# JuliaQuantumControl/Krotov.jl

Hardware: NVIDIA B200
Metric: state_timesteps_per_s (higher is better)
Workload: dtype f64

## Files before the change

krotov.jl_b200/csrc/krotov_cuda.cu:

```cuda
#include <cuda_runtime.h>

#include <algorithm>
#include <chrono>
#include <cmath>
#include <complex>
#include <cstdio>
#include <cstdlib>
#include <cstring>
#include <map>
#include <set>
#include <string>
#include <vector>

#include <thread>

#include "../../include/krotov_cuda.h"
#include "dense_kernel.cuh"
#include "warp_kernel.cuh"
#include "warp2_kernel.cuh"
#include "tiny_kernel.cuh"
#include "kernel_table.h"

using cplx = std::complex<double>;

// ... 961 lines not shown
            dst.assign((size_t)N * h->lpt, cplx(0, 0));
            const cplx *s = reinterpret_cast<const cplx *>(src);
            for (int k = 0; k < N; ++k)
                for (int i = 0; i < d; ++i) dst[(size_t)k * h->lpt + i] = s[(size_t)k * d + i];
        };
        std::vector<cplx> tmp;
        pad_states(pb->psi0, tmp);
        if ((rc = upload(h, h->d_psi0, tmp))) return bail(rc);
        if (h->has_target) {
            pad_states(pb->target, tmp);
            if ((rc = upload(h, h->d_target, tmp))) return bail(rc);
        }
        const size_t slab = (size_t)N * (N_T + 1) * h->lpt * 16;
        h->x_slab = slab / 16;
        if ((rc = dev_alloc(h, h->d_X, slab * (h->rf_wanted ? 2 : 1)))) return bail(rc);
        if (h->store_fw && (rc = dev_alloc(h, h->d_Phi, slab))) return bail(rc);
        if ((rc = dev_alloc(h, h->d_chiT, (size_t)N * h->lpt * 16))) return bail(rc);
        if ((rc = dev_alloc(h, h->d_psif, (size_t)N * h->lpt * 16))) return bail(rc);
        cudaMemcpy(h->d_psif.p, h->d_psi0.p, (size_t)N * h->lpt * 16, cudaMemcpyDeviceToDevice);
        if (h->has_target) {
            std::vector<cplx> tau0(N);
            const cplx *s0 = reinterpret_cast<const cplx *>(pb->psi0), *tg = reinterpret_cast<const cplx *>(pb->target);
            for (int k = 0; k < N; ++k) {
                cplx a(0, 0);
                for (int i = 0; i < d; ++i) a += std::conj(tg[(size_t)k * d + i]) * s0[(size_t)k * d + i];
                tau0[k] = a;
            }
            cudaMemcpy(h->d_tau.p, tau0.data(), (size_t)N * 16, cudaMemcpyHostToDevice);
        }
        h->swept = true;
        if ((rc = dev_alloc(h, h->d_R, ((size_t)N_T * h->nCTA * L + (size_t)N_T * L) * 8))) return bail(rc);
        if ((rc = dev_alloc(h, h->d_acc, (size_t)N_T * L * kr::kFixLimbs * 8))) return bail(rc);
        if (getenv("KROTOV_PROF")) {
            if ((rc = dev_alloc(h, h->d_prof, (size_t)h->nCTA * 8 * 8))) return bail(rc);
            cudaMemset(h->d_prof.p, 0, h->d_prof.bytes);
        }
    } else {
        kr::SparseDesc sd;
        if (path == KROTOV_PATH_SPARSE) {
            sd.W = hs.W; sd.nnz_union = hs.nnz_union; sd.hermitian = hs.hermitian;
            sd.cols = &hs.cols; sd.vals_f = &hs.vals_f; sd.vals_b = &hs.vals_b;
        }
        h->dense = kr::dense_create(h->d, h->N, h->L, h->N_T, h->n_gen, h->Hdense, h->gen_of_traj, pb->psi0,
                                    pb->target, h->store_fw, h->stream, h->err,
                                    path == KROTOV_PATH_SPARSE ? &sd : nullptr);
        if (!h->dense) return bail(KROTOV_ERR_UNSUPPORTED);
        std::vector<cplx>().swap(h->Hdense);
        if (!kr::dense_seed(h->dense, (double2 *)h->d_tau.p, h->err)) return bail(KROTOV_ERR_CUDA);
        h->swept = true;
    }
    if (cudaDeviceSynchronize() != cudaSuccess) return bail(fail(h, KROTOV_ERR_CUDA, "device sync after create failed"));
    *out = h;
    return KROTOV_OK;
}

int krotov_get_info(krotov_handle h, krotov_info *out) {
    if (!h || !out) return KROTOV_ERR_ARG;
    memset(out, 0, sizeof(*out));
    out->struct_size = sizeof(krotov_info);
    out->path = h->path;
    out->ell_width = h->Wt;
    out->nnz_union = h->nnz_union;
    out->grid_blocks = h->nCTA;
    out->block_threads = h->wpc * h->lpt + 32;
    if (h->tiny && h->world == 1 && !h->amp_set) {
        out->grid_blocks = 1;
        out->block_threads = 32;
// ... 505 lines not shown

int krotov_envelope_extremes_device(krotov_handle h, int n_corner, const double *amps, double *e_min, double *e_max) {
    if (!h) return KROTOV_ERR_ARG;
    if (n_corner < 1 || !amps || !e_min || !e_max) return fail(h, KROTOV_ERR_ARG, "bad argument to krotov_envelope_extremes_device");
    if (h->path != KROTOV_PATH_WARP || h->lpt != 32 || !h->d_rawf.p)
        return fail(h, KROTOV_ERR_UNSUPPORTED, "krotov_envelope_extremes_device: persistent kernel path with d <= 32 only");
    cudaSetDevice(h->device);
    int rc;
    const size_t n_out = (size_t)h->n_gen * n_corner;
    if ((rc = dev_alloc(h, h->d_envamps, (size_t)n_corner * h->L * 8 + 16))) return rc;
    if ((rc = dev_alloc(h, h->d_envout, n_out * 16))) return rc;
    KR_CUDA(h, cudaMemcpyAsync(h->d_envamps.p, amps, (size_t)n_corner * h->L * 8, cudaMemcpyHostToDevice, h->stream));
    jacobi_extremes_kernel<<<(unsigned)n_out, 32, 0, h->stream>>>((const double2 *)h->d_rawf.p, (const int *)h->d_cols.p,
                                                                  (const double *)h->d_envamps.p, (double2 *)h->d_envout.p,
                                                                  h->L, h->Wt, h->d, n_corner);
    std::vector<double> out(2 * n_out);
    KR_CUDA(h, cudaMemcpyAsync(out.data(), h->d_envout.p, n_out * 16, cudaMemcpyDeviceToHost, h->stream));
    KR_CUDA(h, cudaStreamSynchronize(h->stream));
    h->launches_total += 1;
    for (int g = 0; g < h->n_gen; ++g) {
        double lo = out[2 * ((size_t)g * n_corner)], hi = out[2 * ((size_t)g * n_corner) + 1];
        for (int c = 1; c < n_corner; ++c) {
            lo = std::min(lo, out[2 * ((size_t)g * n_corner + c)]);
            hi = std::max(hi, out[2 * ((size_t)g * n_corner + c) + 1]);
        }
        e_min[g] = lo;
        e_max[g] = hi;
    }
    return KROTOV_OK;
}

int krotov_get_profile(krotov_handle h, int cta, int64_t *out) {
    if (!h || !out) return KROTOV_ERR_ARG;
    for (int i = 0; i < 8; ++i) out[i] = 0;
    if (!h->d_prof.p) return fail(h, KROTOV_ERR_STATE, "profiling counters are off (set KROTOV_PROF=1 before krotov_create)");
    cudaSetDevice(h->device);
    std::vector<long long> tmp((size_t)h->nCTA * 8);
    KR_CUDA(h, cudaMemcpy(tmp.data(), h->d_prof.p, tmp.size() * 8, cudaMemcpyDeviceToHost));
    if (cta >= h->nCTA) return fail(h, KROTOV_ERR_ARG, "cta out of range");
    for (int c = 0; c < h->nCTA; ++c)
        if (cta < 0 || c == cta)
            for (int i = 0; i < 8; ++i) out[i] = std::max<int64_t>(out[i], tmp[(size_t)c * 8 + i]);
    return KROTOV_OK;
}

struct CommDesc {
    cudaIpcMemHandle_t mh[2];
    cudaIpcMemHandle_t xh;
};
struct CommDescTail {
    int nCTA;
    int n_traj, n_traj_global;
    int rf_ok;
};
static_assert(sizeof(CommDesc) + sizeof(CommDescTail) <= KROTOV_COMM_DESC_BYTES, "descriptor too large");

int krotov_comm_export(krotov_handle h, void *desc) {
    if (!h || !desc) return KROTOV_ERR_ARG;
    cudaSetDevice(h->device);
    CommDesc cd;
    memset(&cd, 0, sizeof(cd));
    for (int par = 0; par < 2; ++par) KR_CUDA(h, cudaIpcGetMemHandle(&cd.mh[par], h->d_mbox[par].p));
    if (h->path == KROTOV_PATH_WARP) KR_CUDA(h, cudaIpcGetMemHandle(&cd.xh, h->d_X.p));
    memset(desc, 0, KROTOV_COMM_DESC_BYTES);
    memcpy(desc, &cd, sizeof(cd));
    CommDescTail tail{h->path == KROTOV_PATH_WARP ? h->nCTA : 0, h->N, h->N_global, rf_eligible(h) ? 1 : 0};
    memcpy((char *)desc + sizeof(cd), &tail, sizeof(tail));
    return KROTOV_OK;
}

int krotov_comm_connect(krotov_handle h, int rank, int world, const void *descs) {
    if (!h || !descs) return KROTOV_ERR_ARG;
    if (world < 1 || world > kr::kMaxRanks || rank < 0 || rank >= world) return fail(h, KROTOV_ERR_ARG, "bad rank/world");
    cudaSetDevice(h->device);
    h->rank = rank;
// ... 54 lines not shown
```

krotov.jl_b200/csrc/warp2_kernel.cuh:

```cuda
#pragma once
#include "warp_kernel.cuh"

namespace kr {

template <int W>
__device__ __forceinline__ void row_dot2(const double2 (&g)[W + 1], const int (&col)[W], const double2 *__restrict__ va,
                                         const double2 *__restrict__ vb, const double2 owna, const double2 ownb,
                                         double &ara, double &aia, double &arb, double &aib) {
    double ra1 = 0.0, ia1 = 0.0, rb1 = 0.0, ib1 = 0.0;
    ara = fma(g[W].x, owna.x, ara);
    ra1 = fma(-g[W].y, owna.y, ra1);
    aia = fma(g[W].x, owna.y, aia);
    ia1 = fma(g[W].y, owna.x, ia1);
    arb = fma(g[W].x, ownb.x, arb);
    rb1 = fma(-g[W].y, ownb.y, rb1);
    aib = fma(g[W].x, ownb.y, aib);
    ib1 = fma(g[W].y, ownb.x, ib1);
#pragma unroll
    for (int s = 0; s < W; ++s) {
        const double2 xa = va[col[s]];
        const double2 xb = vb[col[s]];
        ara = fma(g[s].x, xa.x, ara);
        ra1 = fma(-g[s].y, xa.y, ra1);
        aia = fma(g[s].x, xa.y, aia);
// ... 39 lines not shown
        oai = fma(cj, aia, oai);
        obr = fma(cj, arb, obr);
        obi = fma(cj, aib, obi);
        a2 = a1; b2 = b1;
        a1 = make_double2(ara, aia);
        b1 = make_double2(arb, aib);
        nxtA[lane] = a1;
        nxtB[lane] = b1;
        __syncwarp();
        double2 *t = curA; curA = nxtA; nxtA = t;
        t = curB; curB = nxtB; nxtB = t;
    }
    psia = make_double2(phase.x * oar - phase.y * oai, phase.x * oai + phase.y * oar);
    psib = make_double2(phase.x * obr - phase.y * obi, phase.x * obi + phase.y * obr);
}

template <int W, int LT>
__global__ void __launch_bounds__(256, 1) krotov_warp2_kernel(const __grid_constant__ WarpParams p) {
    constexpr int NT = 1 + LT;
    extern __shared__ __align__(16) unsigned char smem_raw[];
    const int lane = threadIdx.x & 31;
    const int warp = threadIdx.x >> 5;
    constexpr int L = LT;
    const int wpc = p.wpc;
    double2 *vbuf = reinterpret_cast<double2 *>(smem_raw);
    double2 *psis = vbuf + (size_t)wpc * 128;
    double *red = reinterpret_cast<double *>(psis + (size_t)wpc * 64);
    double *eps_s = red + (size_t)L * wpc * 32;
    double *gbuf = eps_s + kMaxCtrl;
    const int nthr_all = (wpc + 1) * 32;
    const int N_T = p.N_T;
    if (warp == wpc) {
        __shared__ __align__(16) WarpParams p_sh;
        comm_warp_run(p, (int)blockIdx.x, L, lane, wpc, nthr_all, red, eps_s, gbuf, &p_sh);
        return;
    }
    const int ka = (blockIdx.x * wpc + warp) * 2, kb = ka + 1;
    const bool live = kb < p.N;
    double2 *bufs = vbuf + (size_t)warp * 128;
    double2 *myps = psis + (size_t)warp * 64;
    int col[W];
#pragma unroll
    for (int s = 0; s < W; ++s) col[s] = p.cols[s * 32 + lane];
    const size_t rowstride = (size_t)(W + 1) * 32;
    double2 P[NT][W + 1];
    double2 g[W + 1];
    const int gi = live ? p.gen_of_traj[ka] : 0;
    const long long t_begin = clock64();

    if (p.mode == 1 && live) {
        const double2 *Pg = p.Pb + (size_t)gi * NT * rowstride;
#pragma unroll
        for (int q = 0; q < NT; ++q) load_row<W>(Pg + q * rowstride, P[q], lane);
        double2 ca, cb;
        if (p.chiT != nullptr) {
            ca = p.chiT[(size_t)ka * 32 + lane];
            cb = p.chiT[(size_t)kb * 32 + lane];
        } else {
            const double2 fa = p.chi_coef[ka], fb = p.chi_coef[kb];
            const double2 ta = p.target[(size_t)ka * 32 + lane], tb = p.target[(size_t)kb * 32 + lane];
            ca = make_double2(fa.x * ta.x - fa.y * ta.y, fa.x * ta.y + fa.y * ta.x);
            cb = make_double2(fb.x * tb.x - fb.y * tb.y, fb.x * tb.y + fb.y * tb.x);
        }
        double2 *Xa = p.X + (size_t)ka * (N_T + 1) * 32, *Xb = p.X + (size_t)kb * (N_T + 1) * 32;
        Xa[(size_t)N_T * 32 + lane] = ca;
        Xb[(size_t)N_T * 32 + lane] = cb;
        myps[lane] = ca;
// ... 92 lines not shown
            for (int l = 0; l < LT; ++l) eps[l] = p.amp_old[(size_t)l * N_T + n];
        }
        const StepMeta fmeta_next =
            load_meta(p.dtc_f, p.m_f, p.phase_f, p.coef_f, p.ndtc_f, p.mmax_f, gi, n + 1 < N_T ? n + 1 : n);
        if (live) {
#pragma unroll
            for (int s = 0; s <= W; ++s) g[s] = P[0][s];
#pragma unroll
            for (int l = 0; l < LT; ++l) {
#pragma unroll
                for (int s = 0; s <= W; ++s) {
                    g[s].x = fma(eps[l], P[l + 1][s].x, g[s].x);
                    g[s].y = fma(eps[l], P[l + 1][s].y, g[s].y);
                }
            }
            cheby_step2<W>(pa, pb, g, col, myps, bufs, fmeta.a, fmeta.m, fmeta.phase, lane);
            myps[lane] = pa;
            myps[32 + lane] = pb;
            __syncwarp();
            if (p.store_fw) {
                const int slot = (p.mode == 1) ? n : n + 1;
                p.Phi[((size_t)ka * (N_T + 1) + slot) * 32 + lane] = pa;
                p.Phi[((size_t)kb * (N_T + 1) + slot) * 32 + lane] = pb;
            }
        }
        fmeta = fmeta_next;
        if (p.prof != nullptr) {
            asm volatile("" ::"d"(pa.x) : "memory");
            t_step += clock64() - ts0;
        }
    }
    if (p.prof != nullptr && warp == 0 && lane == 0) {
        const long long t_end = clock64();
        p.prof[blockIdx.x * 8 + 0] = t_bw_end - t_begin;
        p.prof[blockIdx.x * 8 + 1] = t_end - t_bw_end;
        p.prof[blockIdx.x * 8 + 2] = t_wait_b;
        p.prof[blockIdx.x * 8 + 6] = t_overlap;
        p.prof[blockIdx.x * 8 + 7] = t_step;
    }
    if (live) {
        p.psi_final[(size_t)ka * 32 + lane] = pa;
        p.psi_final[(size_t)kb * 32 + lane] = pb;
        double tar = 0.0, tai = 0.0, tbr = 0.0, tbi = 0.0;
        if (p.target != nullptr) {
            const double2 ta = p.target[(size_t)ka * 32 + lane], tb = p.target[(size_t)kb * 32 + lane];
            tar = ta.x * pa.x + ta.y * pa.y;
            tai = ta.x * pa.y - ta.y * pa.x;
            tbr = tb.x * pb.x + tb.y * pb.y;
            tbi = tb.x * pb.y - tb.y * pb.x;
        }
        tar = warp_sum_xor(tar);
        tai = warp_sum_xor(tai);
        tbr = warp_sum_xor(tbr);
        tbi = warp_sum_xor(tbi);
        if (lane == 0) {
            p.tau[ka] = make_double2(tar, tai);
            p.tau[kb] = make_double2(tbr, tbi);
        }
    }
}

}
```

krotov.jl_b200/csrc/warp_kernel.cuh:

```cuda
#pragma once
#include <cuda_runtime.h>
#include <stdint.h>

namespace kr {

constexpr int kMaxRanks = 8;
constexpr int kMaxCtrl = 8;
constexpr int kAmpMaxDeg = 4;
constexpr unsigned long long kSentinel = 0xFFFFFFFFFFFFFFFFull;

struct WarpParams {
    int d, N, L, N_T, n_gen;
    int wpc;
    int tpw;
    int nCTA;
    int mode;
    int mu_hermitian;
    int store_fw;
    int ndtc_f, ndtc_b, mmax_f, mmax_b;
    const int *gen_of_traj;
    const int *cols;
    const double2 *Pf, *Pb;
    const double *inv_s_f;
    const double *coef_f, *coef_b;
    const int *m_f, *m_b;
    const double2 *phase_f, *phase_b;
    const int *dtc_f, *dtc_b;
    const double *dt;
    const double *alpha;
    const double *eps_old;
    double *eps_new;
    const double *amp_old;
    const double *amp_dfac;
    const double *amp_poly;
    const double *amp_shape;
    double *g_a_int;
    double2 *X;
    double2 *Phi;
    const double2 *psi0;
    const double2 *target;
    const double2 *chiT;
    const double2 *chi_coef;
// ... 295 lines not shown
        mag = mant >> (-shift);
    const unsigned __int128 bias = (unsigned __int128)1 << kFixBiasBit;
    biased = (x < 0.0) ? bias - mag : bias + mag;
    return true;
}

__device__ __forceinline__ double fix_to_double(const unsigned long long w0, const unsigned long long w1,
                                                const unsigned long long w2, const int n) {
    const unsigned long long mask = (1ull << 48) - 1;
    unsigned __int128 sum = (unsigned __int128)(w0 & mask) + ((unsigned __int128)(w1 & mask) << kFixLimbBits) +
                            ((unsigned __int128)(w2 & mask) << (2 * kFixLimbBits));
    const unsigned __int128 bias = (unsigned __int128)n << kFixBiasBit;
    const bool neg = sum < bias;
    const unsigned __int128 mag = neg ? bias - sum : sum - bias;
    const unsigned long long hi = (unsigned long long)(mag >> 64), lo = (unsigned long long)mag;
    double d;
    if (hi == 0) {
        d = __ull2double_rn(lo);
    } else {
        const int sh = 64 - __clzll((long long)hi);
        unsigned long long top = (sh == 64) ? hi : ((hi << (64 - sh)) | (lo >> sh));
        const unsigned long long lost = (sh == 64) ? lo : (lo << (64 - sh));
        if (lost) top |= 1ull;
        d = scalbn(__ull2double_rn(top), sh);
    }
    d = scalbn(d, -kFixFrac);
    return neg ? -d : d;
}

__device__ __forceinline__ void red_add_u64(unsigned long long *p, unsigned long long v) {
    asm volatile("red.relaxed.gpu.global.add.u64 [%0], %1;" ::"l"(p), "l"(v) : "memory");
}

__device__ __forceinline__ bool atomic_grid_sum(unsigned long long *An, const int nCTA, const int L, const int lane,
                                                double (&tot)[kMaxCtrl], int *err_flag, const long long timeout,
                                                const bool wait = true) {
    const int nw = L * kFixLimbs;
    const int myl = lane / kFixLimbs, myj = lane - myl * kFixLimbs;
    double mine = 0.0;
#pragma unroll
    for (int l = 0; l < kMaxCtrl; ++l)
        if (l == myl) mine = tot[l];
    if (lane < nw) {
        unsigned __int128 v;
        const bool ok = fix_from_double(mine, v);
        unsigned long long add = 1ull << 56;
        if (ok)
            add += (unsigned long long)(v >> (myj * kFixLimbBits)) & ((1ull << kFixLimbBits) - 1);
        else
            add += 1ull << 48;
        red_add_u64(An + lane, add);
    }
    if (!wait) return true;
    const long long t0 = clock64();
    int spins = 0;
    unsigned long long w = 0;
    for (;;) {
        if (lane < nw) w = ld_poll_u64<false>(reinterpret_cast<const double *>(An + lane));
        const bool pending = lane < nw && (int)(w >> 56) != nCTA;
        if (!__any_sync(0xffffffffu, pending)) break;
        if ((++spins & 63) == 0) {
            if (clock64() - t0 > timeout || *(volatile int *)err_flag) {
                atomicExch(err_flag, 1);
                break;
            }
        }
    }
    const bool misfit = lane < nw && ((w >> 48) & 0xFF) != 0;
    if (__any_sync(0xffffffffu, misfit)) return false;
    const int src = (lane < L ? lane : 0) * kFixLimbs;
    const unsigned long long w0 = __shfl_sync(0xffffffffu, w, src), w1 = __shfl_sync(0xffffffffu, w, src + 1),
                             w2 = __shfl_sync(0xffffffffu, w, src + 2);
    const double du = fix_to_double(w0, w1, w2, nCTA);
#pragma unroll
    for (int l = 0; l < kMaxCtrl; ++l) tot[l] = __shfl_sync(0xffffffffu, du, l < L ? l : 0);
    return true;
}

constexpr int kXLimbBits = 30, kXLimbs = 4, kXBiasBit = 116, kXMisShift = 41, kXCntShift = 52, kXMaxArrivals = 2047;

__device__ __forceinline__ bool fixx_from_double(const double x, unsigned __int128 &biased) {
    const unsigned long long bits = (unsigned long long)__double_as_longlong(fabs(x));
    const int ebits = (int)(bits >> 52);
    if (ebits >= 1023 + (kXBiasBit - kFixFrac)) return false;
    const unsigned long long mant = (bits & 0xFFFFFFFFFFFFFull) | (ebits ? (1ull << 52) : 0ull);
    const int shift = (ebits ? ebits : 1) - 1075 + kFixFrac;
    unsigned __int128 mag = 0;
    if (shift >= 0)
        mag = (unsigned __int128)mant << shift;
    else if (shift > -64)
        mag = mant >> (-shift);
    const unsigned __int128 bias = (unsigned __int128)1 << kXBiasBit;
    biased = (x < 0.0) ? bias - mag : bias + mag;
    return true;
}

__device__ __forceinline__ double fix_mag_to_double(const unsigned __int128 mag, const bool neg) {
    const unsigned long long hi = (unsigned long long)(mag >> 64), lo = (unsigned long long)mag;
    double d;
    if (hi == 0) {
        d = __ull2double_rn(lo);
    } else {
        const int sh = 64 - __clzll((long long)hi);
        unsigned long long top = (sh == 64) ? hi : ((hi << (64 - sh)) | (lo >> sh));
        const unsigned long long lost = (sh == 64) ? lo : (lo << (64 - sh));
        if (lost) top |= 1ull;
        d = scalbn(__ull2double_rn(top), sh);
    }
    d = scalbn(d, -kFixFrac);
// ... 213 lines not shown
    for (int l = 0; l < kMaxCtrl; ++l) tot[l] = tot_io[l];
    double *Rn = p.R + (size_t)n * L * p.nCTA;
    double *En = p.E + (size_t)n * L;
    if (cta != 0) {
#pragma unroll
        for (int l = 0; l < kMaxCtrl; ++l)
            if (l < L && lane == l) st_relaxed_gpu_f64(Rn + (size_t)l * p.nCTA + cta, tot[l]);
        poll_broadcast(En, L, lane, tot, p.err_flag, p.timeout_cycles);
    } else {
#pragma unroll
        for (int l = 0; l < kMaxCtrl; ++l)
            if (l < L && lane == l) st_relaxed_gpu_f64(Rn + (size_t)l * p.nCTA, tot[l]);
        reducer_gather<false>(Rn, p.nCTA, L, lane, gbuf, tot, p.err_flag, p.timeout_cycles);
#pragma unroll
        for (int l = 0; l < kMaxCtrl; ++l)
            if (l < L && lane == l) st_relaxed_gpu_f64(En + l, tot[l]);
    }
#pragma unroll
    for (int l = 0; l < kMaxCtrl; ++l) tot_io[l] = tot[l];
}

static __device__ __noinline__ double amp_eval_cold(const WarpParams *pp, const int l, const double e, const double shp) {
    double c = e;
    if (pp->amp_poly != nullptr) {
        const double *q = pp->amp_poly + l * (kAmpMaxDeg + 1);
        c = q[kAmpMaxDeg];
#pragma unroll
        for (int d = kAmpMaxDeg - 1; d >= 0; --d) c = fma(c, e, q[d]);
    }
    if (pp->amp_shape != nullptr) c = __dmul_rn(shp, c);
    return c;
}

__device__ __forceinline__ void comm_warp_run(const WarpParams &p, const int cta, const int L, const int lane, const int wpc,
                                              const int nthr_all, double *red, double *eps_s, double *gbuf,
                                              WarpParams *p_sh) {
    const int N_T = p.N_T;
    if (p.mode != 1) return;
    {
        const unsigned long long *src = reinterpret_cast<const unsigned long long *>(&p);
        unsigned long long *dst = reinterpret_cast<unsigned long long *>(p_sh);
        for (int i = lane; i < (int)(sizeof(WarpParams) / 8); i += 32) dst[i] = src[i];
        __syncwarp();
    }
    double ga = 0.0;
    const bool nonlin = p.amp_dfac != nullptr;
    long long c_wait_a = 0, c_reduce = 0, c_gather = 0;
    for (int n = 0; n < N_T; ++n) {
        double a_ln = 0.0, e_old = 0.0, dtn = 0.0, dfac = 1.0, shp = 1.0, a_eff = 0.0;
        if (lane < L) {
            a_ln = p.alpha[(size_t)lane * N_T + n];
            e_old = p.eps_old[(size_t)lane * N_T + n];
            dtn = p.dt[n];
            a_eff = a_ln;
            if (nonlin) {
                dfac = p.amp_dfac[(size_t)lane * N_T + n];
                if (p.amp_shape != nullptr) shp = p.amp_shape[(size_t)lane * N_T + n];
                a_eff = __dmul_rn(a_ln, dfac);
            }
        }
        const long long c0 = clock64();
        bar_sync(1, nthr_all);
        const long long c1 = clock64();
        double tot[kMaxCtrl];
#pragma unroll
        for (int l = 0; l < kMaxCtrl; ++l) {
            double sacc = 0.0;
            if (l < L)
                for (int q = 0; q < wpc; ++q) sacc += red[(size_t)l * wpc * 32 + q * 32 + lane];
            tot[l] = sacc;
        }
#pragma unroll
        for (int o = 16; o > 0; o >>= 1) {
#pragma unroll
            for (int l = 0; l < kMaxCtrl; ++l)
                if (l < L) tot[l] += __shfl_xor_sync(0xffffffffu, tot[l], o);
        }
        const long long c2 = clock64();
        bool summed = p.nCTA == 1 && p.world == 1;
        if (p.world > 1) {
            double tl[kMaxCtrl];
#pragma unroll
            for (int l = 0; l < kMaxCtrl; ++l) tl[l] = tot[l];
            exchange_ranks(p_sh, cta, n, L, lane, tl, gbuf);
#pragma unroll
            for (int l = 0; l < kMaxCtrl; ++l) tot[l] = tl[l];
            summed = true;
        } else if (p.acc != nullptr && p.nCTA > 1) {
            summed = atomic_grid_sum(p.acc + (size_t)n * L * kFixLimbs, p.nCTA, L, lane, tot, p.err_flag, p.timeout_cycles);
            if (!summed && cta == 0 && lane == 0) atomicAdd(p.err_flag + 1, 1);
        }
        if (!summed) {
            double tl[kMaxCtrl];
#pragma unroll
            for (int l = 0; l < kMaxCtrl; ++l) tl[l] = tot[l];
            exchange_gather(p_sh, cta, n, L, lane, tl, gbuf);
#pragma unroll
            for (int l = 0; l < kMaxCtrl; ++l) tot[l] = tl[l];
        }
        const long long c3 = clock64();
        c_wait_a += c1 - c0;
        c_reduce += c2 - c1;
        c_gather += c3 - c2;
        double mine = 0.0;
#pragma unroll
        for (int l = 0; l < kMaxCtrl; ++l)
            if (lane == l) mine = tot[l];
        double e_new = 0.0;
        if (lane < L) {
            const double d_eps = __dmul_rn(a_eff, mine);
            e_new = __dadd_rn(e_old, d_eps);
            double c_new = e_new;
            if (nonlin) c_new = amp_eval_cold(p_sh, lane, e_new, shp);
            eps_s[lane] = c_new;
        }
        bar_arrive(2, nthr_all);
        if (cta == 0 && lane < L) {
            p.eps_new[(size_t)lane * N_T + n] = e_new;
            const double du = nonlin ? __dmul_rn(dfac, mine) : mine;
            ga = __dadd_rn(ga, __dmul_rn(__dmul_rn(a_ln, __dmul_rn(fabs(du), fabs(du))), dtn));
        }
    }
    if (cta == 0 && lane < L) p.g_a_int[lane] = ga;
    if (p.prof != nullptr && lane == 0) {
        p.prof[cta * 8 + 3] = c_wait_a;
        p.prof[cta * 8 + 4] = c_reduce;
        p.prof[cta * 8 + 5] = c_gather;
    }
}

static __device__ __noinline__ void rf_forward_records(const WarpParams *pp, const double2 *rf_ring, unsigned long long *rf_bar,
                                                       int *rf_prog, const int cta, const int warp, const int lane,
                                                       const int n_prod, const int n_fwd) {
    const WarpParams &p = *pp;
    const int N_T = p.N_T, wpc = p.wpc, world = p.rf_world, nCTA = p.nCTA, bw_lo = p.bw_lo;
    const long long timeout = p.timeout_cycles;
    double2 *Xr[kMaxRanks];
#pragma unroll
    for (int r = 0; r < kMaxRanks; ++r) Xr[r] = p.Xr[r];
    const long long t0 = clock64();
    bool dead = false;
    for (int i = 0; i <= N_T && !dead; ++i) {
        for (int w = warp - n_prod; w < n_prod; w += n_fwd) {
            {
                unsigned long long *bar = rf_bar + (size_t)w * kRfRing + (i % kRfRing);
                const unsigned parity = (unsigned)(i / kRfRing) & 1u;
                int tries = 0;
                while (!rf_mbar_try_wait(bar, parity)) {
                    if ((++tries & 63) == 0 && (clock64() - t0 > timeout || *(volatile int *)p.err_flag)) {
                        atomicExch(p.err_flag, 1);
                        dead = true;
                        break;
                    }
                }
            }
            dead = __any_sync(0xffffffffu, dead);
            if (dead) break;
            const double2 v = rf_ring[((size_t)w * kRfRing + (i % kRfRing)) * 32 + lane];
            __syncwarp();
            if (lane == 0) st_release_cta_shared(rf_prog + wpc + w, i + 1);
// ... 81 lines not shown

template <int W, int LT , int MAXTHREADS, int LPT = 32, bool EMUL = false,
          bool RF = false>
__global__ void __launch_bounds__(MAXTHREADS, 1) krotov_warp_kernel(const __grid_constant__ WarpParams p0) {
    const WarpParams &p = select_params<EMUL>(p0);
    const int cta = EMUL ? (int)blockIdx.x - p.cta_base : (int)blockIdx.x;
    constexpr bool PREG = (LT > 0);
    constexpr int NT = PREG ? (1 + LT) : 1;
    extern __shared__ __align__(16) unsigned char smem_raw[];
    const bool is_comm = (int)threadIdx.x >= p.wpc * LPT;
    const int lane = is_comm ? ((int)threadIdx.x - p.wpc * LPT) : ((int)threadIdx.x % LPT);
    const int warp = (int)threadIdx.x / LPT;
    const int gbar = 3 + warp;
    const int L = PREG ? LT : p.L;
    const int wpc = p.wpc, tpw = p.tpw;
    double2 *vbuf = reinterpret_cast<double2 *>(smem_raw);
    double2 *psis = vbuf + (size_t)wpc * 2 * LPT;
    double *red = reinterpret_cast<double *>(psis + (size_t)wpc * tpw * LPT);
    double *eps_s = red + (size_t)L * wpc * LPT;
    double *gbuf = eps_s + kMaxCtrl;
    double2 *chibufs = reinterpret_cast<double2 *>(gbuf + kMaxCtrl * 160);
    double2 *rf_ring = chibufs + (size_t)wpc * LPT;
    unsigned long long *rf_bar = reinterpret_cast<unsigned long long *>(rf_ring + (size_t)wpc * kRfRing * 32);
    int *rf_prog = reinterpret_cast<int *>(rf_bar + (size_t)wpc * kRfRing);
    const int nthr_all = wpc * LPT + 32;
    const int N_T = p.N_T;
    const bool rf_fwd = RF && LPT == 32 && p.rf_world > 1 && p.rf_fwd != 0 && p.mode == 1;
    if (rf_fwd) {
        if ((int)threadIdx.x < 2 * wpc) rf_prog[threadIdx.x] = 0;
        if ((int)threadIdx.x < wpc * kRfRing) rf_mbar_init(rf_bar + threadIdx.x, 1);
        __syncthreads();
    }

    if constexpr (RF) {
        if (is_comm) return;
    }
    if (is_comm) {
        __shared__ __align__(16) WarpParams p_sh;
        comm_warp_run(p, cta, L, lane, wpc * (LPT / 32), nthr_all, red, eps_s, gbuf, &p_sh);
        return;
    }

    const int gw = cta * wpc + warp;
    const int kbase = gw * tpw;
    double2 *bufA = vbuf + (size_t)warp * 2 * LPT;
    double2 *bufB = bufA + LPT;
    double2 *mypsi = psis + (size_t)warp * tpw * LPT;

    int col[W];
#pragma unroll
    for (int s = 0; s < W; ++s) col[s] = p.cols[s * LPT + lane];

    const size_t rowstride = (size_t)(W + 1) * LPT;
    double2 P[NT][W + 1];
    double2 g[W + 1];

    const long long t_begin = clock64();
    long long t_wait_b = 0, t_overlap = 0, t_step = 0;
    const bool rf = RF && p.rf_world > 1;
    const int n_prod = !rf ? 0
                       : p.rf_pack ? min(p.rf_pack, max(0, p.bw_hi - p.bw_lo - cta * p.rf_pack))
                                   : min(wpc, max(0, (p.bw_hi - p.bw_lo - cta + p.nCTA - 1) / p.nCTA));
    const int n_fwd = wpc - n_prod;
    const bool use_fwd = rf_fwd && n_prod > 0 && n_fwd > 0;
    const int vw = RF ? (warp * max(1, p.rf_stride)) % wpc : warp;
    if constexpr (RF)
        if (p.mode == 1 && use_fwd && vw >= n_prod) rf_forward_records(&p, rf_ring, rf_bar, rf_prog, cta, vw, lane, n_prod, n_fwd);
    if (p.mode == 1 && (RF || !p.skip_bw)) {
        for (int t = 0; t < tpw; ++t) {
            int k = kbase + t;
            if constexpr (RF) if (rf) {
                const int tl = p.rf_pack ? (vw < p.rf_pack ? cta * p.rf_pack + vw : p.N) : vw * p.nCTA + cta;
// ... 52 lines not shown
                    for (int l = 0; l < L; ++l) {
                        const double e = p.amp_old[(size_t)l * N_T + n];
                        const double2 *Pl = Pg + (size_t)(l + 1) * rowstride;
#pragma unroll
                        for (int s = 0; s <= W; ++s) {
                            const double2 v = Pl[s * LPT + lane];
                            g[s].x = fma(e, v.x, g[s].x);
                            g[s].y = fma(e, v.y, g[s].y);
                        }
                    }
                }
                if constexpr (RF) {
                    rfp.peek();
                    chi = cheby_step<W, LPT>(chi, g, col, rfp.v0, bufA, bufB, meta.a, meta.m, meta.phase, lane, gbar);
                } else {
                    chi = cheby_step<W, LPT>(chi, g, col, mypsi + t * LPT, bufA, bufB, meta.a, meta.m, meta.phase, lane, gbar);
                }
                meta = meta_next;
#pragma unroll
                for (int l = 0; l < kMaxCtrl; ++l) e_cur[l] = e_next[l];
                if constexpr (RF) {
                    rfp.template put<LPT>(p, n, chi, lane, gbar);
                } else {
                    mypsi[t * LPT + lane] = chi;
                    grp_sync<LPT>(gbar);
                    Xk[(size_t)n * LPT + lane] = chi;
                }
            }
        }
        if constexpr (RF)
            if (rf) rf_rank_barrier<LPT>(&p, cta, warp, lane, gbar);
    }
    if constexpr (RF) {
        if (p.prof != nullptr && warp == 0 && lane == 0) p.prof[cta * 8 + 0] = clock64() - t_begin;
        return;
    }

    const long long t_bw_end = clock64();
    double2 psi_reg = make_double2(0.0, 0.0);
    for (int t = 0; t < tpw; ++t) {
        const int k = kbase + t;
        double2 v = make_double2(0.0, 0.0);
        if (k < p.N) {
            v = p.psi0[(size_t)k * LPT + lane];
            if (p.store_fw) p.Phi[(size_t)k * (N_T + 1) * LPT + lane] = v;
        }
        mypsi[t * LPT + lane] = v;
        if (t == 0) psi_reg = v;
    }
    grp_sync<LPT>(gbar);
    const int k0 = kbase;
    const int g0 = (k0 < p.N) ? p.gen_of_traj[k0] : 0;
    if (PREG && k0 < p.N) {
        const double2 *Pg = p.Pf + (size_t)g0 * (1 + L) * rowstride;
#pragma unroll
        for (int q = 0; q < NT; ++q) load_row<W, LPT>(Pg + q * rowstride, P[q], lane);
    }
    const double inv_s0 = (k0 < p.N) ? p.inv_s_f[g0] : 0.0;
    StepMeta fmeta = load_meta(p.dtc_f, p.m_f, p.phase_f, p.coef_f, p.ndtc_f, p.mmax_f, g0, 0);
    double2 chi_next = make_double2(0.0, 0.0);
    if (p.mode == 1 && k0 < p.N) chi_next = p.X[(size_t)k0 * (N_T + 1) * LPT + lane];
    const bool FAST = PREG && tpw == 1 && p.mode == 1 && p.mu_hermitian != 0;
    double2 *chibuf = chibufs + (size_t)warp * LPT;
    double2 xi[PREG ? (LT > 0 ? LT : 1) : 1];
    double2 wv[PREG ? NT : 1];
    if (PREG && FAST) {
        chibuf[lane] = chi_next;
// ... 18 lines not shown
                if (k0 < p.N) {
#pragma unroll
                    for (int l = 0; l < NT - 1; ++l)
                        part[l] = -inv_s0 * fma(xi[l].x, psi_reg.x, xi[l].y * psi_reg.y);
                }
            } else
            for (int t = 0; t < tpw; ++t) {
                const int k = kbase + t;
                if (k >= p.N) break;
                const int gi = (t == 0) ? g0 : p.gen_of_traj[k];
                const double inv_s = (t == 0) ? inv_s0 : p.inv_s_f[gi];
                const double2 psi = (tpw == 1) ? psi_reg : mypsi[t * LPT + lane];
                const double2 chi = (t == 0) ? chi_next : p.X[((size_t)k * (N_T + 1) + n) * LPT + lane];
                if (PREG) {
#pragma unroll
                    for (int l = 0; l < NT - 1; ++l) {
                        double wr = 0.0, wi = 0.0;
                        row_dot<W>(P[l + 1], col, mypsi + t * LPT, psi, wr, wi);
                        part[l] = fma(inv_s, fma(chi.x, wr, chi.y * wi), part[l]);
                    }
                } else {
                    const double2 *Pg = p.Pf + (size_t)gi * (1 + L) * rowstride;
                    for (int l = 0; l < L; ++l) {
                        load_row<W, LPT>(Pg + (size_t)(l + 1) * rowstride, g, lane);
                        double wr = 0.0, wi = 0.0;
                        row_dot<W>(g, col, mypsi + t * LPT, psi, wr, wi);
                        part[l] = fma(inv_s, fma(chi.x, wr, chi.y * wi), part[l]);
                    }
                }
            }
#pragma unroll
            for (int l = 0; l < (PREG ? LT : kMaxCtrl); ++l)
                if (l < L) red[(size_t)l * wpc * LPT + warp * LPT + lane] = part[l];
            bar_arrive(1, nthr_all);
            const long long w0 = clock64();
            t_overlap += w0 - ts0;
            if (n + 1 < N_T && k0 < p.N) chi_next = p.X[((size_t)k0 * (N_T + 1) + n + 1) * LPT + lane];
            if (PREG && FAST && k0 < p.N) {
#pragma unroll
                for (int q = 0; q < NT; ++q) {
                    double wr = 0.0, wi = 0.0;
                    row_dot<W>(P[q], col, mypsi, psi_reg, wr, wi);
                    wv[q] = make_double2(wr, wi);
                }
                chibuf[lane] = chi_next;
                grp_sync<LPT>(gbar);
#pragma unroll
                for (int l = 0; l < NT - 1; ++l) {
                    double wr = 0.0, wi = 0.0;
                    row_dot<W>(P[l + 1], col, chibuf, chi_next, wr, wi);
                    xi[l] = make_double2(wr, wi);
                }
                grp_sync<LPT>(gbar);
            }
            bar_sync(2, nthr_all);
#pragma unroll
            for (int l = 0; l < (PREG ? LT : kMaxCtrl); ++l)
                if (l < L) eps[l] = eps_s[l];
            if (p.prof != nullptr) {
                asm volatile("" ::"d"(eps[0]) : "memory");
                t_wait_b += clock64() - w0;
            }
        } else {
#pragma unroll
            for (int l = 0; l < (PREG ? LT : kMaxCtrl); ++l)
                if (l < L) eps[l] = p.amp_old[(size_t)l * N_T + n];
        }
        const StepMeta fmeta_next =
            load_meta(p.dtc_f, p.m_f, p.phase_f, p.coef_f, p.ndtc_f, p.mmax_f, g0, n + 1 < N_T ? n + 1 : n);
        for (int t = 0; t < tpw; ++t) {
// ... 3 lines not shown
            const StepMeta sm = (t == 0) ? fmeta : load_meta(p.dtc_f, p.m_f, p.phase_f, p.coef_f, p.ndtc_f, p.mmax_f, gi, n);
            if (PREG) {
#pragma unroll
                for (int s = 0; s <= W; ++s) g[s] = P[0][s];
#pragma unroll
                for (int l = 0; l < NT - 1; ++l) {
#pragma unroll
                    for (int s = 0; s <= W; ++s) {
                        g[s].x = fma(eps[l], P[l + 1][s].x, g[s].x);
                        g[s].y = fma(eps[l], P[l + 1][s].y, g[s].y);
                    }
                }
            } else {
                const double2 *Pg = p.Pf + (size_t)gi * (1 + L) * rowstride;
                load_row<W, LPT>(Pg, g, lane);
                for (int l = 0; l < L; ++l) {
                    const double2 *Pl = Pg + (size_t)(l + 1) * rowstride;
#pragma unroll
                    for (int s = 0; s <= W; ++s) {
                        const double2 v = Pl[s * LPT + lane];
                        g[s].x = fma(eps[l], v.x, g[s].x);
                        g[s].y = fma(eps[l], v.y, g[s].y);
                    }
                }
            }
            double2 psi = (tpw == 1) ? psi_reg : mypsi[t * LPT + lane];
            if (PREG && FAST) {
                double v1r = wv[0].x, v1i = wv[0].y;
#pragma unroll
                for (int l = 0; l < NT - 1; ++l) {
                    v1r = fma(eps[l], wv[l + 1].x, v1r);
                    v1i = fma(eps[l], wv[l + 1].y, v1i);
                }
                psi = cheby_step_from_v1<W, LPT>(psi, make_double2(0.5 * v1r, 0.5 * v1i), g, col, bufA, bufB, sm.a, sm.m,
                                            sm.phase, lane, gbar);
            } else {
                psi = cheby_step<W, LPT>(psi, g, col, mypsi + t * LPT, bufA, bufB, sm.a, sm.m, sm.phase, lane, gbar);
            }
            mypsi[t * LPT + lane] = psi;
            if (t == 0) psi_reg = psi;
            grp_sync<LPT>(gbar);
            if (p.store_fw) {
                const int slot = (p.mode == 1) ? n : n + 1;
                p.Phi[((size_t)k * (N_T + 1) + slot) * LPT + lane] = psi;
            }
        }
        fmeta = fmeta_next;
        if (p.prof != nullptr) {
            asm volatile("" ::"d"(psi_reg.x) : "memory");
            t_step += clock64() - ts0;
        }
    }

    if (p.prof != nullptr && warp == 0 && lane == 0) {
        const long long t_end = clock64();
        if (!p.skip_bw) p.prof[cta * 8 + 0] = t_bw_end - t_begin;
        p.prof[cta * 8 + 1] = t_end - t_bw_end;
        p.prof[cta * 8 + 2] = t_wait_b;
        p.prof[cta * 8 + 6] = t_overlap;
        p.prof[cta * 8 + 7] = t_step;
    }
    for (int t = 0; t < tpw; ++t) {
        const int k = kbase + t;
        if (k >= p.N) break;
        const double2 psi = mypsi[t * LPT + lane];
        p.psi_final[(size_t)k * LPT + lane] = psi;
        double tr = 0.0, ti = 0.0;
        if (p.target != nullptr) {
            const double2 tg = p.target[(size_t)k * LPT + lane];
            tr = tg.x * psi.x + tg.y * psi.y;
            ti = tg.x * psi.y - tg.y * psi.x;
        }
        tr = warp_sum_xor(tr);
        ti = warp_sum_xor(ti);
        if (LPT > 32) {
            grp_sync<LPT>(gbar);
            if ((lane & 31) == 0) bufA[lane >> 5] = make_double2(tr, ti);
            grp_sync<LPT>(gbar);
            tr = 0.0;
            ti = 0.0;
            for (int q = 0; q < LPT / 32; ++q) {
                tr += bufA[q].x;
                ti += bufA[q].y;
            }
        }
        if (lane == 0) p.tau[k] = make_double2(tr, ti);
    }
}

}
```

krotov.jl_b200/engine.py:

```python
from __future__ import annotations

import ctypes as C

import numpy as np

from . import _lib as B


def _ptr(a):
    return None if a is None else a.ctypes.data_as(C.c_void_p)


class KrotovCuda:
    def __init__(self, *, tlist, H0, Hc, gen_of_traj, psi0, target=None, weight=None, update_shape, lambda_a,
                 functional=B.CHI_HOST, n_traj_global=0, store_fw=False, device=0, force_path=0, csr=False,
                 replicated_forward=False):
        lib = B.lib()
        self._lib = lib
        self._h = C.c_void_p()
        tlist = np.ascontiguousarray(tlist, np.float64)
        psi0 = np.ascontiguousarray(psi0, np.complex128)
        N, d = psi0.shape
        n_gen = len(H0)
        L = len(Hc[0])
# ... 118 lines not shown
        c = np.ascontiguousarray(coef, np.complex128).reshape(self.N)
        self._check(self._lib.krotov_set_chi_coeffs(self._h, _ptr(c)))

    def iterate(self, guess_pulses, out_pulses=None):
        g = np.ascontiguousarray(guess_pulses, np.float64).reshape(self.L, self.N_T)
        out = np.empty((self.L, self.N_T), np.float64) if out_pulses is None else out_pulses
        ga = np.empty(self.L, np.float64)
        self._check(self._lib.krotov_iterate(self._h, _ptr(g), _ptr(out), _ptr(ga)))
        return out, ga

    def states(self):
        out = np.empty((self.N, self.d), np.complex128)
        self._check(self._lib.krotov_get_states(self._h, _ptr(out)))
        return out

    def tau(self):
        out = np.empty(self.N, np.complex128)
        self._check(self._lib.krotov_get_tau(self._h, _ptr(out)))
        return out

    def storage(self, which, k, n0=0, n1=None):
        n1 = self.N_T + 1 if n1 is None else n1
        out = np.empty((n1 - n0, self.d), np.complex128)
        self._check(self._lib.krotov_get_storage(self._h, int(which), int(k), int(n0), int(n1), _ptr(out)))
        return out

    def envelope_extremes(self, corners):
        amps = np.ascontiguousarray(corners, np.float64).reshape(-1, self.L)
        lo, hi = np.empty(self.n_gen, np.float64), np.empty(self.n_gen, np.float64)
        self._check(self._lib.krotov_envelope_extremes_device(self._h, amps.shape[0], _ptr(amps), _ptr(lo), _ptr(hi)))
        return lo, hi

    def profile(self, cta=-1):
        out = np.zeros(8, np.int64)
        self._check(self._lib.krotov_get_profile(self._h, int(cta), _ptr(out)))
        names = ["backward", "forward", "wait_pulse", "comm_wait_partials", "comm_reduce", "comm_gather", "overlap", "fw_step_total"]
        return dict(zip(names, out.tolist()))

    def comm_export(self):
        buf = (C.c_ubyte * B.COMM_DESC_BYTES)()
        self._check(self._lib.krotov_comm_export(self._h, buf))
        return bytes(buf)

    def comm_connect(self, rank, world, descs):
        blob = b"".join(descs)
        assert len(blob) == world * B.COMM_DESC_BYTES
        buf = (C.c_ubyte * len(blob)).from_buffer_copy(blob)
        self._check(self._lib.krotov_comm_connect(self._h, int(rank), int(world), buf))


class KrotovCudaGroup:

    def __init__(self, engines, bounds, gens, replicated=False):
        self.engines, self.bounds, self.gens = list(engines), list(bounds), [np.asarray(g, int) for g in gens]
        self.replicated = bool(replicated)
        e0 = self.engines[0]
        self._lib = e0._lib
        self.N = e0.N if replicated else sum(e.N for e in self.engines)
        self.d, self.L, self.N_T = e0.d, e0.L, e0.N_T
        self.n_gen = len(self.gens[0]) if replicated else sum(len(g) for g in self.gens)
        self.world = len(self.engines)
        self.pulses_all = None
        arr = (C.c_void_p * self.world)(*[e._h for e in self.engines])
        self._handles = arr
        rc = self._lib.krotov_group_connect(arr, self.world)
        if rc != B.KROTOV_OK:
            raise B.KrotovCudaError(rc, "; ".join(self._lib.krotov_last_error(e._h).decode() for e in self.engines))

    def close(self):
# ... 77 lines not shown
```

Baseline: 333.8 million.

## Add handoff profiling slots, preload comm reduction, gate compute on send barrier

Widens the per-CTA profile record to 16 slots and adds handoff timestamps (skew, send, sum, update, release, SM id) that are recorded only when profiling is on. Separately, the comm warp's shared-memory partial reduction is unrolled over a compile-time maximum warp count, so all loads are issued before summing. A new named barrier makes compute warps wait until the comm warp has posted its atomic contribution before continuing, on the preloaded-register single-device multi-CTA path. The barrier could add stall on the compute warps while the unrolled reduction shortens the comm warp's critical section.

New measurement: 348.5 million (median of 6 runs). 1.04x the previous value.

```diff
diff --git a/krotov.jl_b200/csrc/krotov_cuda.cu b/krotov.jl_b200/csrc/krotov_cuda.cu
--- a/krotov.jl_b200/csrc/krotov_cuda.cu
+++ b/krotov.jl_b200/csrc/krotov_cuda.cu
@@ -1017,7 +1017,7 @@
         if ((rc = dev_alloc(h, h->d_R, ((size_t)N_T * h->nCTA * L + (size_t)N_T * L) * 8))) return bail(rc);
         if ((rc = dev_alloc(h, h->d_acc, (size_t)N_T * L * kr::kFixLimbs * 8))) return bail(rc);
         if (getenv("KROTOV_PROF")) {
-            if ((rc = dev_alloc(h, h->d_prof, (size_t)h->nCTA * 8 * 8))) return bail(rc);
+            if ((rc = dev_alloc(h, h->d_prof, (size_t)h->nCTA * kr::kProfSlots * 8))) return bail(rc);
             cudaMemset(h->d_prof.p, 0, h->d_prof.bytes);
         }
     } else {
@@ -1589,15 +1589,15 @@
 
 int krotov_get_profile(krotov_handle h, int cta, int64_t *out) {
     if (!h || !out) return KROTOV_ERR_ARG;
-    for (int i = 0; i < 8; ++i) out[i] = 0;
+    for (int i = 0; i < kr::kProfSlots; ++i) out[i] = 0;
     if (!h->d_prof.p) return fail(h, KROTOV_ERR_STATE, "profiling counters are off (set KROTOV_PROF=1 before krotov_create)");
     cudaSetDevice(h->device);
-    std::vector<long long> tmp((size_t)h->nCTA * 8);
+    std::vector<long long> tmp((size_t)h->nCTA * kr::kProfSlots);
     KR_CUDA(h, cudaMemcpy(tmp.data(), h->d_prof.p, tmp.size() * 8, cudaMemcpyDeviceToHost));
     if (cta >= h->nCTA) return fail(h, KROTOV_ERR_ARG, "cta out of range");
     for (int c = 0; c < h->nCTA; ++c)
         if (cta < 0 || c == cta)
-            for (int i = 0; i < 8; ++i) out[i] = std::max<int64_t>(out[i], tmp[(size_t)c * 8 + i]);
+            for (int i = 0; i < kr::kProfSlots; ++i) out[i] = std::max<int64_t>(out[i], tmp[(size_t)c * kr::kProfSlots + i]);
     return KROTOV_OK;
 }
 
diff --git a/krotov.jl_b200/csrc/warp2_kernel.cuh b/krotov.jl_b200/csrc/warp2_kernel.cuh
--- a/krotov.jl_b200/csrc/warp2_kernel.cuh
+++ b/krotov.jl_b200/csrc/warp2_kernel.cuh
@@ -95,7 +95,7 @@
     const int N_T = p.N_T;
     if (warp == wpc) {
         __shared__ __align__(16) WarpParams p_sh;
-        comm_warp_run(p, (int)blockIdx.x, L, lane, wpc, nthr_all, red, eps_s, gbuf, &p_sh);
+        comm_warp_run<7>(p, (int)blockIdx.x, L, lane, wpc, nthr_all, red, eps_s, gbuf, &p_sh, nullptr, false);
         return;
     }
     const int ka = (blockIdx.x * wpc + warp) * 2, kb = ka + 1;
@@ -254,11 +254,11 @@
     }
     if (p.prof != nullptr && warp == 0 && lane == 0) {
         const long long t_end = clock64();
-        p.prof[blockIdx.x * 8 + 0] = t_bw_end - t_begin;
-        p.prof[blockIdx.x * 8 + 1] = t_end - t_bw_end;
-        p.prof[blockIdx.x * 8 + 2] = t_wait_b;
-        p.prof[blockIdx.x * 8 + 6] = t_overlap;
-        p.prof[blockIdx.x * 8 + 7] = t_step;
+        p.prof[blockIdx.x * kProfSlots + 0] = t_bw_end - t_begin;
+        p.prof[blockIdx.x * kProfSlots + 1] = t_end - t_bw_end;
+        p.prof[blockIdx.x * kProfSlots + 2] = t_wait_b;
+        p.prof[blockIdx.x * kProfSlots + 6] = t_overlap;
+        p.prof[blockIdx.x * kProfSlots + 7] = t_step;
     }
     if (live) {
         p.psi_final[(size_t)ka * 32 + lane] = pa;
diff --git a/krotov.jl_b200/csrc/warp_kernel.cuh b/krotov.jl_b200/csrc/warp_kernel.cuh
--- a/krotov.jl_b200/csrc/warp_kernel.cuh
+++ b/krotov.jl_b200/csrc/warp_kernel.cuh
@@ -8,6 +8,9 @@
 constexpr int kMaxCtrl = 8;
 constexpr int kAmpMaxDeg = 4;
 constexpr unsigned long long kSentinel = 0xFFFFFFFFFFFFFFFFull;
+constexpr int kProfSlots = 16;
+constexpr int kHpRel = 32, kHpFirst = 33, kHpSlots = 34;
+constexpr int kBarSent = 14;
 
 struct WarpParams {
     int d, N, L, N_T, n_gen;
@@ -369,9 +372,7 @@
     asm volatile("red.relaxed.gpu.global.add.u64 [%0], %1;" ::"l"(p), "l"(v) : "memory");
 }
 
-__device__ __forceinline__ bool atomic_grid_sum(unsigned long long *An, const int nCTA, const int L, const int lane,
-                                                double (&tot)[kMaxCtrl], int *err_flag, const long long timeout,
-                                                const bool wait = true) {
+__device__ __forceinline__ void atomic_grid_add(unsigned long long *An, const int L, const int lane, const double (&tot)[kMaxCtrl]) {
     const int nw = L * kFixLimbs;
     const int myl = lane / kFixLimbs, myj = lane - myl * kFixLimbs;
     double mine = 0.0;
@@ -388,7 +389,11 @@
             add += 1ull << 48;
         red_add_u64(An + lane, add);
     }
-    if (!wait) return true;
+}
+
+__device__ __forceinline__ bool atomic_grid_poll(unsigned long long *An, const int nCTA, const int L, const int lane,
+                                                 double (&tot)[kMaxCtrl], int *err_flag, const long long timeout) {
+    const int nw = L * kFixLimbs;
     const long long t0 = clock64();
     int spins = 0;
     unsigned long long w = 0;
@@ -412,6 +417,14 @@
 #pragma unroll
     for (int l = 0; l < kMaxCtrl; ++l) tot[l] = __shfl_sync(0xffffffffu, du, l < L ? l : 0);
     return true;
+}
+
+__device__ __forceinline__ bool atomic_grid_sum(unsigned long long *An, const int nCTA, const int L, const int lane,
+                                                double (&tot)[kMaxCtrl], int *err_flag, const long long timeout,
+                                                const bool wait = true) {
+    atomic_grid_add(An, L, lane, tot);
+    if (!wait) return true;
+    return atomic_grid_poll(An, nCTA, L, lane, tot, err_flag, timeout);
 }
 
 constexpr int kXLimbBits = 30, kXLimbs = 4, kXBiasBit = 116, kXMisShift = 41, kXCntShift = 52, kXMaxArrivals = 2047;
@@ -691,9 +704,10 @@
     return c;
 }
 
+template <int MAXW>
 __device__ __forceinline__ void comm_warp_run(const WarpParams &p, const int cta, const int L, const int lane, const int wpc,
                                               const int nthr_all, double *red, double *eps_s, double *gbuf,
-                                              WarpParams *p_sh) {
+                                              WarpParams *p_sh, long long *hp, const bool send_gate) {
     const int N_T = p.N_T;
     if (p.mode != 1) return;
     {
@@ -704,7 +718,7 @@
     }
     double ga = 0.0;
     const bool nonlin = p.amp_dfac != nullptr;
-    long long c_wait_a = 0, c_reduce = 0, c_gather = 0;
+    long long c_wait_a = 0, c_reduce = 0, c_gather = 0, h_skew = 0, h_send = 0, h_sum = 0, h_update = 0;
     for (int n = 0; n < N_T; ++n) {
         double a_ln = 0.0, e_old = 0.0, dtn = 0.0, dfac = 1.0, shp = 1.0, a_eff = 0.0;
         if (lane < L) {
@@ -722,12 +736,28 @@
         bar_sync(1, nthr_all);
         const long long c1 = clock64();
         double tot[kMaxCtrl];
-#pragma unroll
-        for (int l = 0; l < kMaxCtrl; ++l) {
-            double sacc = 0.0;
-            if (l < L)
-                for (int q = 0; q < wpc; ++q) sacc += red[(size_t)l * wpc * 32 + q * 32 + lane];
-            tot[l] = sacc;
+        if constexpr (MAXW > 0) {
+            double v[kMaxCtrl][MAXW];
+#pragma unroll
+            for (int l = 0; l < kMaxCtrl; ++l)
+#pragma unroll
+                for (int q = 0; q < MAXW; ++q) v[l][q] = (l < L && q < wpc) ? red[(size_t)l * wpc * 32 + q * 32 + lane] : 0.0;
+#pragma unroll
+            for (int l = 0; l < kMaxCtrl; ++l) {
+                double sacc = 0.0;
+#pragma unroll
+                for (int q = 0; q < MAXW; ++q)
+                    if (l < L && q < wpc) sacc += v[l][q];
+                tot[l] = sacc;
+            }
+        } else {
+#pragma unroll
+            for (int l = 0; l < kMaxCtrl; ++l) {
+                double sacc = 0.0;
+                if (l < L)
+                    for (int q = 0; q < wpc; ++q) sacc += red[(size_t)l * wpc * 32 + q * 32 + lane];
+                tot[l] = sacc;
+            }
         }
 #pragma unroll
         for (int o = 16; o > 0; o >>= 1) {
@@ -736,6 +766,7 @@
                 if (l < L) tot[l] += __shfl_xor_sync(0xffffffffu, tot[l], o);
         }
         const long long c2 = clock64();
+        long long t_seen = 0;
         bool summed = p.nCTA == 1 && p.world == 1;
         if (p.world > 1) {
             double tl[kMaxCtrl];
@@ -746,7 +777,22 @@
             for (int l = 0; l < kMaxCtrl; ++l) tot[l] = tl[l];
             summed = true;
         } else if (p.acc != nullptr && p.nCTA > 1) {
-            summed = atomic_grid_sum(p.acc + (size_t)n * L * kFixLimbs, p.nCTA, L, lane, tot, p.err_flag, p.timeout_cycles);
+            unsigned long long *An = p.acc + (size_t)n * L * kFixLimbs;
+            atomic_grid_add(An, L, lane, tot);
+            const long long t_sent = clock64();
+            if (send_gate) bar_arrive(kBarSent, nthr_all);
+            summed = atomic_grid_poll(An, p.nCTA, L, lane, tot, p.err_flag, p.timeout_cycles);
+            t_seen = clock64();
+            if (hp != nullptr) {
+                long long t_lo = hp[0], t_hi = hp[0];
+                for (int q = 1; q < wpc; ++q) {
+                    t_lo = min(t_lo, hp[q]);
+                    t_hi = max(t_hi, hp[q]);
+                }
+                h_skew += t_hi - t_lo;
+                h_send += t_sent - t_hi;
+                h_sum += t_seen - t_sent;
+            }
             if (!summed && cta == 0 && lane == 0) atomicAdd(p.err_flag + 1, 1);
         }
         if (!summed) {
@@ -773,6 +819,11 @@
             if (nonlin) c_new = amp_eval_cold(p_sh, lane, e_new, shp);
             eps_s[lane] = c_new;
         }
+        if (hp != nullptr) {
+            const long long t_rel = clock64();
+            if (t_seen != 0) h_update += t_rel - t_seen;
+            if (lane == 0) hp[kHpRel] = t_rel;
+        }
         bar_arrive(2, nthr_all);
         if (cta == 0 && lane < L) {
             p.eps_new[(size_t)lane * N_T + n] = e_new;
@@ -782,9 +833,16 @@
     }
     if (cta == 0 && lane < L) p.g_a_int[lane] = ga;
     if (p.prof != nullptr && lane == 0) {
-        p.prof[cta * 8 + 3] = c_wait_a;
-        p.prof[cta * 8 + 4] = c_reduce;
-        p.prof[cta * 8 + 5] = c_gather;
+        p.prof[cta * kProfSlots + 3] = c_wait_a;
+        p.prof[cta * kProfSlots + 4] = c_reduce;
+        p.prof[cta * kProfSlots + 5] = c_gather;
+        p.prof[cta * kProfSlots + 8] = h_skew;
+        p.prof[cta * kProfSlots + 9] = h_send;
+        p.prof[cta * kProfSlots + 10] = h_sum;
+        p.prof[cta * kProfSlots + 11] = h_update;
+        unsigned smid;
+        asm volatile("mov.u32 %0, %%smid;" : "=r"(smid));
+        p.prof[cta * kProfSlots + 13] = smid;
     }
 }
 
@@ -932,12 +990,21 @@
         __syncthreads();
     }
 
+    __shared__ long long hp_sh[kHpSlots];
+    long long *hp = p.prof != nullptr ? hp_sh : nullptr;
+    if (hp != nullptr) {
+        if (threadIdx.x == 0) hp_sh[kHpFirst] = 0;
+        __syncthreads();
+    }
     if constexpr (RF) {
         if (is_comm) return;
     }
+    const bool send_gate = PREG && LPT == 32 && !RF && tpw == 1 && p.mode == 1 && p.mu_hermitian != 0 && p.world == 1 &&
+                           p.nCTA > 1 && p.acc != nullptr;
     if (is_comm) {
         __shared__ __align__(16) WarpParams p_sh;
-        comm_warp_run(p, cta, L, lane, wpc * (LPT / 32), nthr_all, red, eps_s, gbuf, &p_sh);
+        comm_warp_run<PREG ? MAXTHREADS / 32 - 1 : 0>(p, cta, L, lane, wpc * (LPT / 32), nthr_all, red, eps_s, gbuf, &p_sh, hp,
+                                                      send_gate);
         return;
     }
 
@@ -1056,7 +1123,7 @@
             if (rf) rf_rank_barrier<LPT>(&p, cta, warp, lane, gbar);
     }
     if constexpr (RF) {
-        if (p.prof != nullptr && warp == 0 && lane == 0) p.prof[cta * 8 + 0] = clock64() - t_begin;
+        if (p.prof != nullptr && warp == 0 && lane == 0) p.prof[cta * kProfSlots + 0] = clock64() - t_begin;
         return;
     }
 
@@ -1141,10 +1208,12 @@
 #pragma unroll
             for (int l = 0; l < (PREG ? LT : kMaxCtrl); ++l)
                 if (l < L) red[(size_t)l * wpc * LPT + warp * LPT + lane] = part[l];
+            if (hp != nullptr && (threadIdx.x & 31) == 0) hp[threadIdx.x >> 5] = clock64();
             bar_arrive(1, nthr_all);
             const long long w0 = clock64();
             t_overlap += w0 - ts0;
             if (n + 1 < N_T && k0 < p.N) chi_next = p.X[((size_t)k0 * (N_T + 1) + n + 1) * LPT + lane];
+            if (send_gate) bar_sync(kBarSent, nthr_all);
             if (PREG && FAST && k0 < p.N) {
 #pragma unroll
                 for (int q = 0; q < NT; ++q) {
@@ -1214,6 +1283,10 @@
                     v1r = fma(eps[l], wv[l + 1].x, v1r);
                     v1i = fma(eps[l], wv[l + 1].y, v1i);
                 }
+                if (hp != nullptr && threadIdx.x == 0) {
+                    asm volatile("" ::"d"(v1r), "d"(v1i), "d"(g[0].x), "d"(g[W].y) : "memory");
+                    hp[kHpFirst] += clock64() - hp[kHpRel];
+                }
                 psi = cheby_step_from_v1<W, LPT>(psi, make_double2(0.5 * v1r, 0.5 * v1i), g, col, bufA, bufB, sm.a, sm.m,
                                             sm.phase, lane, gbar);
             } else {
@@ -1236,11 +1309,12 @@
 
     if (p.prof != nullptr && warp == 0 && lane == 0) {
         const long long t_end = clock64();
-        if (!p.skip_bw) p.prof[cta * 8 + 0] = t_bw_end - t_begin;
-        p.prof[cta * 8 + 1] = t_end - t_bw_end;
-        p.prof[cta * 8 + 2] = t_wait_b;
-        p.prof[cta * 8 + 6] = t_overlap;
-        p.prof[cta * 8 + 7] = t_step;
+        if (!p.skip_bw) p.prof[cta * kProfSlots + 0] = t_bw_end - t_begin;
+        p.prof[cta * kProfSlots + 1] = t_end - t_bw_end;
+        p.prof[cta * kProfSlots + 2] = t_wait_b;
+        p.prof[cta * kProfSlots + 6] = t_overlap;
+        p.prof[cta * kProfSlots + 7] = t_step;
+        p.prof[cta * kProfSlots + 12] = hp[kHpFirst];
     }
     for (int t = 0; t < tpw; ++t) {
         const int k = kbase + t;
diff --git a/krotov.jl_b200/engine.py b/krotov.jl_b200/engine.py
--- a/krotov.jl_b200/engine.py
+++ b/krotov.jl_b200/engine.py
@@ -174,9 +174,10 @@
         return lo, hi
 
     def profile(self, cta=-1):
-        out = np.zeros(8, np.int64)
+        out = np.zeros(16, np.int64)
         self._check(self._lib.krotov_get_profile(self._h, int(cta), _ptr(out)))
-        names = ["backward", "forward", "wait_pulse", "comm_wait_partials", "comm_reduce", "comm_gather", "overlap", "fw_step_total"]
+        names = ["backward", "forward", "wait_pulse", "comm_wait_partials", "comm_reduce", "comm_gather", "overlap", "fw_step_total",
+                 "hand_skew", "hand_send", "hand_sum", "hand_update", "hand_release", "smid", "unused14", "unused15"]
         return dict(zip(names, out.tolist()))
 
     def comm_export(self):
```
